# liuyuan-pal/Gen6D

Measured on AMD Instinct MI355X. Metric: query images/sec (detect+select+3x refine), 64 ref views, higher is better.
Workload: dtype f32

## Files before the change

### gen6d_amd/csrc/corr16_geom.h

```cpp
#pragma once
#include "conv16w_geom.h"

namespace corr16g {

constexpr int BM = c16g::BM;
constexpr int NW = 11;
constexpr int STAGE = 42 * 1024;
constexpr int PIECE = 1024;
constexpr int NPL = STAGE / PIECE;
constexpr int TAP_BYTES = 2048;
constexpr int RING = 3;
constexpr int RED_LD = 33;
constexpr int LDS_BYTES = 2 * STAGE;
static_assert((STAGE / 64 + 15) / 16 <= NPL, "the largest patch pick_tile admits (STAGE / 64 rows) fits NPL pieces");
static_assert(4 * BM * RED_LD * 4 <= LDS_BYTES, "the final reduction's four partial tiles fit the two stages");

struct Tile { int tw_log2, tiles_x, tpi, swa, swd; };
C16G_HD Tile pick_tile(int H, int W, int K) {
  double best = 1e30; int btw = 0;
  for (int tw = 32; tw >= 4; tw >>= 1) {
    const int th = BM / tw;
    if ((th + K - 1) * (tw + K - 1) > STAGE / 64) continue;
    const double waste = (double)((W + tw - 1) / tw * tw) * ((H + th - 1) / th * th) / ((double)W * H);
    if (waste < best - 1e-9) { best = waste; btw = tw; }
  }
  if (!btw) return {-1, 0, 0, 0, 0};
  int l2 = 0; while ((1 << l2) < btw) ++l2;
  const int th = BM / btw, tx = (W + btw - 1) / btw;
  return {l2, tx, tx * ((H + th - 1) / th), btw == 32 ? 2 : (btw == 16 ? 1 : 0), btw <= 8 ? 1 : 0};
}

struct Patch { int tw_log2, K, swa, swd, PW, P, NI; };
C16G_HD Patch patch_of(int tw_log2, int K, int swa, int swd) {
  const int PW = (1 << tw_log2) + K - 1, P = ((BM >> tw_log2) + K - 1) * PW;
  return {tw_log2, K, swa, swd, PW, P, (P + 15) >> 4};
}
struct Origin { int n, y0, x0; };
C16G_HD Origin tile_origin(const Patch& g, int tiles_x, int tpi, int t) {
  const int n = t / tpi, r = t - n * tpi, ty = r / tiles_x, tx = r - ty * tiles_x;
  return {n, ty * (BM >> g.tw_log2), tx * (1 << g.tw_log2)};
}

struct Piece { int prow, pcol, y, x, L; bool in_patch; };
C16G_HD Piece piece_of(const Patch& g, const Origin& o, int k, int lane) {
  const int q = k * 16 + (lane >> 2), R = g.K >> 1;
  const int prow = q / g.PW, pcol = q - prow * g.PW;
  return {prow, pcol, o.y0 - R + prow, o.x0 - R + pcol, (lane & 3) ^ (((pcol >> g.swa) + prow * g.swd) & 3), k < g.NI && q < g.P};
}
C16G_HD bool in_map(const Piece& pc, int H, int W) { return pc.y >= 0 && pc.y < H && pc.x >= 0 && pc.x < W; }
C16G_HD unsigned slot_bytes(int L, bool pairs, int Cin) { return pairs ? (unsigned)((L >> 1) * Cin * 2 + (L & 1) * 16) : (unsigned)(L * 16); }

C16G_HD void frag_base(const Patch& g, int r, int& qb, int& fe) {
  const int py = r >> g.tw_log2, px = r & ((1 << g.tw_log2) - 1);
  qb = (py * g.PW + px) * 64; fe = px + py * g.swd;
}
C16G_HD int tap_addr(const Patch& g, int qb, int fe, int fhalf, int ky, int kx, int stage) {
  const int so = stage * STAGE + ky * (g.PW * 64) + kx * 64, sw = ((fe + kx) >> g.swa) + ky * g.swd;
  return qb + so + (((fhalf ^ sw) & 3) << 4);
}

C16G_HD int wave_taps(int K, int wv) { return (K * K - wv + NW - 1) / NW; }
C16G_HD void first_tap(int K, int wv, int& ky, int& kx) { ky = wv / K; kx = wv - ky * K; }
C16G_HD void next_tap(int K, int& ky, int& kx) { kx += NW; while (kx >= K) { kx -= K; ++ky; } }
C16G_HD long filter_advance(int K, int wv, int& wtap) {
  wtap += NW;
  if (wtap < K * K) return NW * TAP_BYTES;
  const long d = (long)(K * K - wtap + NW + wv) * TAP_BYTES;
  wtap = wv;
  return d;
}

}
```

### gen6d_amd/csrc/detector.hip

```cpp
#include "g6d_common.h"

namespace {

struct LevelStats { float mu[3], sigma[3]; };

__global__ void assemble_kernel(const float* __restrict__ s0, const float* __restrict__ s1, const float* __restrict__ s2,
                                int hc, int wc, int rfn, LevelStats st, float clip, int hs, int ws, int scale_idx,
                                int nch, float* __restrict__ stacked) {
  const long long total = (long long)hs * ws * rfn;
  const long long i = blockIdx.x * (long long)blockDim.x + threadIdx.x;
  if (i >= total) return;
  s0 += (size_t)blockIdx.y * hc * wc * rfn; s1 += (size_t)blockIdx.y * (hc >> 1) * (wc >> 1) * rfn;
  s2 += (size_t)blockIdx.y * (hc >> 2) * (wc >> 2) * rfn; stacked += (size_t)blockIdx.y * total * nch;
  const int r = (int)(i % rfn); const int pix = (int)(i / rfn);
  const int x = pix % ws, y = pix / ws;
  const float ry = (float)hc / (float)hs, rx = (float)wc / (float)ws;
  float sy = ry * (y + 0.5f) - 0.5f; if (sy < 0.f) sy = 0.f;
  float sx = rx * (x + 0.5f) - 0.5f; if (sx < 0.f) sx = 0.f;
  const int y0 = (int)sy, x0 = (int)sx;
  const int y1 = y0 + (y0 < hc - 1), x1 = x0 + (x0 < wc - 1);
  const float ly = sy - y0, lx = sx - x0, hy = 1.f - ly, hx = 1.f - lx;
  const float* src[3] = {s0, s1, s2};
  float* dst = stacked + ((size_t)pix * rfn + r) * nch + 3 * scale_idx;
#pragma unroll
  for (int l = 0; l < 3; ++l) {
    const int wl = wc >> l;
    const float mu = st.mu[l], sg = st.sigma[l];
    auto tap = [&](int yy, int xx) {
      float v = src[l][((size_t)(yy >> l) * wl + (xx >> l)) * rfn + r];
      v = (v - mu) / sg;
      return fminf(fmaxf(v, -clip), clip);
    };
    dst[l] = hy * (hx * tap(y0, x0) + lx * tap(y0, x1)) + ly * (hx * tap(y1, x0) + lx * tap(y1, x1));
  }
}

__device__ __forceinline__ int enc_f(float f) { int b = __float_as_int(f); return b >= 0 ? b : b ^ 0x7fffffff; }
__device__ __forceinline__ float dec_f(int b) { return __int_as_float(b >= 0 ? b : b ^ 0x7fffffff); }

template <int NCH>
__global__ void __launch_bounds__(256) score_mlp_max_kernel(const float* __restrict__ stacked, int P, int rfn,
                                                            const float* __restrict__ w0, const float* __restrict__ b0,
                                                            const float* __restrict__ w1, const float* __restrict__ b1,
                                                            float* __restrict__ out, int ppb) {
  extern __shared__ int smax[];
  const int pl = threadIdx.x / rfn, r = threadIdx.x % rfn;
  const int pix = blockIdx.x * ppb + pl;
  for (int i = threadIdx.x; i < ppb * 64; i += 256) smax[i] = enc_f(-INFINITY);
  __syncthreads();
  if (pl < ppb && pix < P) {
    float in[NCH];
    const float* src = stacked + ((size_t)pix * rfn + r) * NCH;
#pragma unroll
    for (int k = 0; k < NCH; ++k) in[k] = src[k];
    typedef float f2 __attribute__((ext_vector_type(2)));
    static_assert(NCH % 2 == 0, "channel pairs");
    f2 inp[NCH / 2];
#pragma unroll
    for (int k = 0; k < NCH / 2; ++k) inp[k] = f2{in[2 * k], in[2 * k + 1]};
    f2 hp[32];
#pragma unroll
    for (int o = 0; o < 64; ++o) {
      f2 a = {b0[o], 0.f};
#pragma unroll
      for (int k = 0; k < NCH / 2; ++k) a = __builtin_elementwise_fma(inp[k], *reinterpret_cast<const f2*>(w0 + o * NCH + 2 * k), a);
      const float v = fmaxf(a.x + a.y, 0.f);
      if (o & 1) hp[o >> 1].y = v; else hp[o >> 1].x = v;
    }
    for (int o = 0; o < 64; ++o) {
      f2 a = {b1[o], 0.f};
#pragma unroll
      for (int k = 0; k < 32; ++k) a = __builtin_elementwise_fma(hp[k], *reinterpret_cast<const f2*>(w1 + o * 64 + 2 * k), a);
      atomicMax(&smax[pl * 64 + o], enc_f(a.x + a.y));
    }
  }
  __syncthreads();
  for (int i = threadIdx.x; i < ppb * 64; i += 256) {
    const int p2 = blockIdx.x * ppb + i / 64;
    if (p2 < P) out[(size_t)p2 * 64 + (i & 63)] = dec_f(smax[i]);
  }
}

__global__ void __launch_bounds__(256) decode_kernel(const float* __restrict__ scores, int ld_s,
                                                     const float* __restrict__ offset, int ld_o,
                                                     const float* __restrict__ scale, int ld_c, int hs, int ws,
                                                     float pool_ratio, float* __restrict__ result) {
  __shared__ float bv[256];
  __shared__ int bi[256];
  const int n = hs * ws;
  scores += (size_t)blockIdx.x * n * ld_s; offset += (size_t)blockIdx.x * n * ld_o; scale += (size_t)blockIdx.x * n * ld_c;
  result += blockIdx.x * 5;
  float best = -INFINITY; int idx = 0x7fffffff;
  for (int i = threadIdx.x; i < n; i += 256) {
    float v = scores[(size_t)i * ld_s];
    if (v > best || (v == best && i < idx)) { best = v; idx = i; }
  }
  bv[threadIdx.x] = best; bi[threadIdx.x] = idx;
  __syncthreads();
  for (int s = 128; s > 0; s >>= 1) {
    if (threadIdx.x < s) {
      float v = bv[threadIdx.x + s]; int j = bi[threadIdx.x + s];
      if (v > bv[threadIdx.x] || (v == bv[threadIdx.x] && j < bi[threadIdx.x])) { bv[threadIdx.x] = v; bi[threadIdx.x] = j; }
    }
    __syncthreads();
  }
  if (threadIdx.x == 0) {
    const int id = bi[0] == 0x7fffffff ? 0 : bi[0];
    const int x = id % ws, y = id / ws;
    result[0] = ((float)x + offset[(size_t)id * ld_o] + 0.5f) * pool_ratio - 0.5f;
    result[1] = ((float)y + offset[(size_t)id * ld_o + 1] + 0.5f) * pool_ratio - 0.5f;
    result[2] = exp2f(scale[(size_t)id * ld_c]);
    result[3] = (float)x; result[4] = (float)y;
  }
}


struct PyrArgs { const float* src; int planes, H, W, n; int h[4], w[4]; long long first[5]; float* dst[4]; };

#define PYR_PL 4
template <int VEC>
__global__ void resize_pyramid_kernel(const PyrArgs a) {
  const unsigned total = (unsigned)a.first[a.n];
  for (unsigned long i64 = blockIdx.x * blockDim.x + threadIdx.x; i64 < total; i64 += (unsigned long)gridDim.x * blockDim.x) {
    const unsigned i = (unsigned)i64;
    int k = 0;
#pragma unroll
    for (int j = 1; j < 4; ++j) k = (j < a.n && i >= (unsigned)a.first[j]) ? j : k;
    const unsigned l = i - (unsigned)a.first[k];
    const int h = a.h[k], w = a.w[k], wv = w / VEC;
    const int xq = (int)(l % (unsigned)wv); const unsigned t = l / (unsigned)wv;
    const int y = (int)(t % (unsigned)h), pg = (int)(t / (unsigned)h);
    const float ry = (float)a.H / (float)h, rx = (float)a.W / (float)w;
    float sy = ry * (y + 0.5f) - 0.5f; if (sy < 0.f) sy = 0.f;
    const int y0 = min((int)sy, a.H - 1);
    const int y1 = y0 + (y0 < a.H - 1);
    const float ly = sy - y0, hy = 1.f - ly;
    int x0[VEC], x1[VEC]; float lx[VEC];
#pragma unroll
    for (int e = 0; e < VEC; ++e) {
      const int x = xq * VEC + e;
      float sx = rx * (x + 0.5f) - 0.5f; if (sx < 0.f) sx = 0.f;
      x0[e] = min((int)sx, a.W - 1);
      x1[e] = x0[e] + (x0[e] < a.W - 1);
      lx[e] = sx - x0[e];
    }
    const size_t sstride = (size_t)a.H * a.W, dstride = (size_t)h * w;
    const int pl0 = pg * PYR_PL;
    const float* r0 = a.src + (size_t)pl0 * sstride + (size_t)y0 * a.W;
    const float* r1 = a.src + (size_t)pl0 * sstride + (size_t)y1 * a.W;
    float t00[PYR_PL][VEC], t01[PYR_PL][VEC], t10[PYR_PL][VEC], t11[PYR_PL][VEC];
#pragma unroll
    for (int p_ = 0; p_ < PYR_PL; ++p_) {
      const size_t o = (size_t)min(p_, a.planes - 1 - pl0) * sstride;
#pragma unroll
      for (int e = 0; e < VEC; ++e) { t00[p_][e] = r0[o + x0[e]]; t01[p_][e] = r0[o + x1[e]]; t10[p_][e] = r1[o + x0[e]]; t11[p_][e] = r1[o + x1[e]]; }
    }
    float* d = a.dst[k] + (size_t)pl0 * dstride + (size_t)y * w + xq * VEC;
#pragma unroll
    for (int p_ = 0; p_ < PYR_PL; ++p_) {
      if (pl0 + p_ >= a.planes) break;
      float v[VEC];
#pragma unroll
      for (int e = 0; e < VEC; ++e) {
        const float hx = 1.f - lx[e];
        v[e] = hy * (hx * t00[p_][e] + lx[e] * t01[p_][e]) + ly * (hx * t10[p_][e] + lx[e] * t11[p_][e]);
      }
      if constexpr (VEC == 4) *reinterpret_cast<f32x4*>(d + p_ * dstride) = f32x4{v[0], v[1], v[2], v[3]};
      else d[p_ * dstride] = v[0];
    }
  }
}
}

#define STREAM(s) reinterpret_cast<hipStream_t>(s)

extern "C" int g6d_detector_assemble(const float* s0, const float* s1, const float* s2, int hc, int wc, int rfn,
                                     const float* mu_sigma, float clip, int hs, int ws, int scale_idx, int nch,
                                     float* stacked, int batch, g6d_stream_t stream) {
  if (!s0 || !s1 || !s2 || !mu_sigma || !stacked || hc <= 0 || wc <= 0 || (hc & 3) || (wc & 3) || rfn <= 0 || hs <= 0 || ws <= 0 ||
      scale_idx < 0 || 3 * scale_idx + 3 > nch || batch < 1 || batch > 65535) {
    g6d_set_error("detector_assemble: bad args (level-0 map must be a multiple of 4, hs and ws positive)"); return G6D_EINVAL;
  }
  LevelStats st;
  for (int l = 0; l < 3; ++l) { st.mu[l] = mu_sigma[2 * l]; st.sigma[l] = mu_sigma[2 * l + 1]; }
  const long long total = (long long)hs * ws * rfn;
  hipLaunchKernelGGL(assemble_kernel, dim3((unsigned)((total + 255) / 256), batch), dim3(256), 0, STREAM(stream), s0, s1, s2, hc,
                     wc, rfn, st, clip, hs, ws, scale_idx, nch, stacked);
  return g6d_check_launch("detector_assemble");
}

extern "C" int g6d_detector_score_mlp_max(const float* stacked, int P, int rfn, int nch, const float* w0, const float* b0,
                                          const float* w1, const float* b1, float* out, g6d_stream_t stream) {
  if (!stacked || !w0 || !b0 || !w1 || !b1 || !out || P <= 0 || rfn <= 0 || rfn > 256 || nch != 12) {
    g6d_set_error("detector_score_mlp_max: bad args (rfn <= 256, nch == 12)"); return G6D_EINVAL;
  }
  const int ppb = 256 / rfn;
  hipLaunchKernelGGL(score_mlp_max_kernel<12>, dim3((P + ppb - 1) / ppb), dim3(256), (size_t)ppb * 64 * sizeof(int),
                     STREAM(stream), stacked, P, rfn, w0, b0, w1, b1, out, ppb);
  return g6d_check_launch("detector_score_mlp_max");
}

extern "C" int g6d_detector_decode(const float* scores, int ld_s, const float* offset, int ld_o, const float* scale,
                                   int ld_c, int hs, int ws, int pool_ratio, float* result, int batch, g6d_stream_t stream) {
  if (!scores || !offset || !scale || !result || hs <= 0 || ws <= 0 || batch < 1) { g6d_set_error("detector_decode: bad args"); return G6D_EINVAL; }
  hipLaunchKernelGGL(decode_kernel, dim3(batch), dim3(256), 0, STREAM(stream), scores, ld_s, offset, ld_o, scale, ld_c, hs, ws,
                     (float)pool_ratio, result);
  return g6d_check_launch("detector_decode");
}

extern "C" int g6d_resize_bilinear_pyramid(const float* src, int planes, int H, int W, int nscale, const int* hs, const int* ws,
                                           float* const* dsts, g6d_stream_t stream) {
  if (!src || !hs || !ws || !dsts || planes <= 0 || H <= 0 || W <= 0 || nscale < 1 || nscale > 4) {
    g6d_set_error("resize_bilinear_pyramid: bad args (1..4 destination sizes)"); return G6D_EINVAL;
  }
  PyrArgs a = {};
  a.src = src; a.planes = planes; a.H = H; a.W = W; a.n = nscale;
  bool vec = true;
  for (int k = 0; k < nscale; ++k)
    if (hs[k] <= 0 || ws[k] <= 0 || !dsts[k]) { g6d_set_error("resize_bilinear_pyramid: bad destination"); return G6D_EINVAL; }
    else vec = vec && (ws[k] & 3) == 0 && g6d_aligned16(dsts[k]);
  long long tot = 0;
  for (int k = 0; k < nscale; ++k) {
    a.h[k] = hs[k]; a.w[k] = ws[k]; a.dst[k] = dsts[k]; a.first[k] = tot;
    tot += (long long)((planes + PYR_PL - 1) / PYR_PL) * hs[k] * (vec ? ws[k] / 4 : ws[k]);
  }
  for (int k = nscale; k < 5; ++k) a.first[k] = tot;
  if (tot >= (1ll << 32)) { g6d_set_error("resize_bilinear_pyramid: more than 2^32 work items"); return G6D_EINVAL; }
  const long long blocks = (tot + 255) / 256;
  const dim3 grid((unsigned)(blocks < 65536 * 8 ? blocks : 65536 * 8));
  if (vec) hipLaunchKernelGGL(resize_pyramid_kernel<4>, grid, dim3(256), 0, STREAM(stream), a);
  else hipLaunchKernelGGL(resize_pyramid_kernel<1>, grid, dim3(256), 0, STREAM(stream), a);
  return g6d_check_launch("resize_bilinear_pyramid");
}
```

Measured before the change: 361.3.

## Run detector score MLP on MFMA with wave-level segmented max reduction

Rewrites the per-pixel two-layer score MLP so each wave processes 32-row tiles with 32x32x2 f32 MFMA instructions. Weights are held in registers and biases are staged in LDS. The per-pixel max over reference views is done with DPP/swizzle or shuffle-based segmented reductions before the LDS atomics, so far fewer atomics are issued. Each block now covers more pixels (up to 1024/rfn, capped at 128). The cost is heavy register use and a more complex reduction path. A live_taps helper is also added to the correlation geometry header, but nothing calls it yet.

```diff
diff --git a/gen6d_amd/csrc/corr16_geom.h b/gen6d_amd/csrc/corr16_geom.h
--- a/gen6d_amd/csrc/corr16_geom.h
+++ b/gen6d_amd/csrc/corr16_geom.h
@@ -59,6 +59,19 @@
   return qb + so + (((fhalf ^ sw) & 3) << 4);
 }
 
+struct Live { int ky0, ky1, kx0, kx1; };
+C16G_HD Live live_taps(const Patch& g, const Origin& o, int H, int W, int mt) {
+  const int R = g.K >> 1, tw = 1 << g.tw_log2;
+  const int ya = o.y0 + ((32 * mt) >> g.tw_log2), xa = o.x0 + ((32 * mt) & (tw - 1));
+  int yb = o.y0 + ((32 * mt + 31) >> g.tw_log2), xb = o.x0 + ((32 * mt + 31) & (tw - 1));
+  if (ya >= H || xa >= W) return {0, 0, 0, 0};
+  if (yb > H - 1) yb = H - 1;
+  if (xb > W - 1) xb = W - 1;
+  const int ky0 = R - yb > 0 ? R - yb : 0, ky1 = H + R - ya < g.K ? H + R - ya : g.K;
+  const int kx0 = R - xb > 0 ? R - xb : 0, kx1 = W + R - xa < g.K ? W + R - xa : g.K;
+  return {ky0, ky1, kx0, kx1};
+}
+
 C16G_HD int wave_taps(int K, int wv) { return (K * K - wv + NW - 1) / NW; }
 C16G_HD void first_tap(int K, int wv, int& ky, int& kx) { ky = wv / K; kx = wv - ky * K; }
 C16G_HD void next_tap(int K, int& ky, int& kx) { kx += NW; while (kx >= K) { kx -= K; ++ky; } }
diff --git a/gen6d_amd/csrc/detector.hip b/gen6d_amd/csrc/detector.hip
--- a/gen6d_amd/csrc/detector.hip
+++ b/gen6d_amd/csrc/detector.hip
@@ -38,47 +38,108 @@
 __device__ __forceinline__ int enc_f(float f) { int b = __float_as_int(f); return b >= 0 ? b : b ^ 0x7fffffff; }
 __device__ __forceinline__ float dec_f(int b) { return __int_as_float(b >= 0 ? b : b ^ 0x7fffffff); }
 
+template <int CTRL>
+__device__ __forceinline__ int max_dpp(int v) { return max(v, __builtin_amdgcn_update_dpp(v, v, CTRL, 0xf, 0xf, false)); }
+
 template <int NCH>
-__global__ void __launch_bounds__(256) score_mlp_max_kernel(const float* __restrict__ stacked, int P, int rfn,
+__global__ void __launch_bounds__(256, 2) score_mlp_max_kernel(const float* __restrict__ stacked, int P, int rfn,
                                                             const float* __restrict__ w0, const float* __restrict__ b0,
                                                             const float* __restrict__ w1, const float* __restrict__ b1,
                                                             float* __restrict__ out, int ppb) {
+  static_assert(NCH == 12, "layer 0 is six K pairs: channels s and 6 + s");
   extern __shared__ int smax[];
-  const int pl = threadIdx.x / rfn, r = threadIdx.x % rfn;
-  const int pix = blockIdx.x * ppb + pl;
-  for (int i = threadIdx.x; i < ppb * 64; i += 256) smax[i] = enc_f(-INFINITY);
+  float* bias = reinterpret_cast<float*>(smax + ppb * 64);
+  const int tid = threadIdx.x, lane = tid & 63, wv = __builtin_amdgcn_readfirstlane(tid >> 6), n = lane & 31, h = lane >> 5;
+  const int p0 = blockIdx.x * ppb, np = min(P - p0, ppb), nrows = np * rfn;
+  const float* rows = stacked + (size_t)p0 * rfn * NCH;
+  for (int i = tid; i < ppb * 64; i += 256) smax[i] = enc_f(-INFINITY);
+  if (tid < 128) bias[tid] = tid < 64 ? b0[tid] : b1[tid - 64];
+  auto unit = [&](int i) { return 8 * (i >> 2) + 4 * h + (i & 3); };
+  float wa[2][6], wb[2][2][16];
+#pragma unroll
+  for (int ht = 0; ht < 2; ++ht)
+#pragma unroll
+    for (int s = 0; s < 6; ++s) wa[ht][s] = w0[(32 * ht + n) * NCH + 6 * h + s];
+#pragma unroll
+  for (int ot = 0; ot < 2; ++ot)
+#pragma unroll
+    for (int ht = 0; ht < 2; ++ht)
+#pragma unroll
+      for (int i = 0; i < 16; ++i) wb[ot][ht][i] = w1[(32 * ot + n) * 64 + 32 * ht + unit(i)];
   __syncthreads();
-  if (pl < ppb && pix < P) {
-    float in[NCH];
-    const float* src = stacked + ((size_t)pix * rfn + r) * NCH;
-#pragma unroll
-    for (int k = 0; k < NCH; ++k) in[k] = src[k];
+  const int ntiles = (nrows + 31) >> 5;
+#pragma unroll 1
+  for (int t = wv; t < ntiles; t += 4) {
+    const int row = 32 * t + n;
+    const bool valid = row < nrows;
     typedef float f2 __attribute__((ext_vector_type(2)));
-    static_assert(NCH % 2 == 0, "channel pairs");
-    f2 inp[NCH / 2];
-#pragma unroll
-    for (int k = 0; k < NCH / 2; ++k) inp[k] = f2{in[2 * k], in[2 * k + 1]};
-    f2 hp[32];
-#pragma unroll
-    for (int o = 0; o < 64; ++o) {
-      f2 a = {b0[o], 0.f};
-#pragma unroll
-      for (int k = 0; k < NCH / 2; ++k) a = __builtin_elementwise_fma(inp[k], *reinterpret_cast<const f2*>(w0 + o * NCH + 2 * k), a);
-      const float v = fmaxf(a.x + a.y, 0.f);
-      if (o & 1) hp[o >> 1].y = v; else hp[o >> 1].x = v;
-    }
-    for (int o = 0; o < 64; ++o) {
-      f2 a = {b1[o], 0.f};
-#pragma unroll
-      for (int k = 0; k < 32; ++k) a = __builtin_elementwise_fma(hp[k], *reinterpret_cast<const f2*>(w1 + o * 64 + 2 * k), a);
-      atomicMax(&smax[pl * 64 + o], enc_f(a.x + a.y));
-    }
+    f2 x[3] = {{0.f, 0.f}, {0.f, 0.f}, {0.f, 0.f}};
+    if (valid) {
+      const f2* src = reinterpret_cast<const f2*>(rows + (size_t)row * NCH + 6 * h);
+#pragma unroll
+      for (int k = 0; k < 3; ++k) x[k] = src[k];
+    }
+    f32x16 hid[2], o[2];
+#pragma unroll
+    for (int ht = 0; ht < 2; ++ht)
+#pragma unroll
+      for (int i = 0; i < 16; ++i) { hid[ht][i] = bias[32 * ht + unit(i)]; o[ht][i] = bias[64 + 32 * ht + unit(i)]; }
+#pragma unroll
+    for (int s = 0; s < 6; ++s)
+#pragma unroll
+      for (int ht = 0; ht < 2; ++ht) hid[ht] = __builtin_amdgcn_mfma_f32_32x32x2f32(wa[ht][s], s & 1 ? x[s >> 1].y : x[s >> 1].x, hid[ht], 0, 0, 0);
+#pragma unroll
+    for (int ht = 0; ht < 2; ++ht)
+#pragma unroll
+      for (int i = 0; i < 16; ++i) {
+        const float hv = fmaxf(hid[ht][i], 0.f);
+#pragma unroll
+        for (int ot = 0; ot < 2; ++ot) o[ot] = __builtin_amdgcn_mfma_f32_32x32x2f32(wb[ot][ht][i], hv, o[ot], 0, 0, 0);
+      }
+    int e[2][16];
+#pragma unroll
+    for (int ot = 0; ot < 2; ++ot)
+#pragma unroll
+      for (int i = 0; i < 16; ++i) e[ot][i] = enc_f(valid ? o[ot][i] : -INFINITY);
+    const int pl = row / rfn;
+    bool head;
+    if (32 * t + 31 < nrows && (32 * t) / rfn == (32 * t + 31) / rfn) {
+#pragma unroll
+      for (int ot = 0; ot < 2; ++ot)
+#pragma unroll
+        for (int i = 0; i < 16; ++i) {
+          int v = e[ot][i];
+          v = max_dpp<0xb1>(v);
+          v = max_dpp<0x4e>(v);
+          v = max_dpp<0x141>(v);
+          v = max_dpp<0x140>(v);
+          e[ot][i] = max(v, __builtin_amdgcn_ds_swizzle(v, 0x401f));
+        }
+      head = n == 0;
+    } else {
+      for (int d = 1; d < 32; d <<= 1) {
+        if (d >= rfn) break;
+        const int pd = __shfl_down(valid ? pl : -1, d, 32);
+        const bool take = (n + d < 32) & (pd == pl);
+#pragma unroll
+        for (int ot = 0; ot < 2; ++ot)
+#pragma unroll
+          for (int i = 0; i < 16; ++i) {
+            const int other = __shfl_down(e[ot][i], d, 32);
+            if (take) e[ot][i] = max(e[ot][i], other);
+          }
+      }
+      const int before = __shfl_up(pl, 1, 32);
+      head = valid && (n == 0 || before != pl);
+    }
+    if (head)
+#pragma unroll
+      for (int ot = 0; ot < 2; ++ot)
+#pragma unroll
+        for (int i = 0; i < 16; ++i) atomicMax(&smax[pl * 64 + 32 * ot + unit(i)], e[ot][i]);
   }
   __syncthreads();
-  for (int i = threadIdx.x; i < ppb * 64; i += 256) {
-    const int p2 = blockIdx.x * ppb + i / 64;
-    if (p2 < P) out[(size_t)p2 * 64 + (i & 63)] = dec_f(smax[i]);
-  }
+  for (int i = tid; i < np * 64; i += 256) out[(size_t)p0 * 64 + i] = dec_f(smax[i]);
 }
 
 __global__ void __launch_bounds__(256) decode_kernel(const float* __restrict__ scores, int ld_s,
@@ -194,8 +255,8 @@
   if (!stacked || !w0 || !b0 || !w1 || !b1 || !out || P <= 0 || rfn <= 0 || rfn > 256 || nch != 12) {
     g6d_set_error("detector_score_mlp_max: bad args (rfn <= 256, nch == 12)"); return G6D_EINVAL;
   }
-  const int ppb = 256 / rfn;
-  hipLaunchKernelGGL(score_mlp_max_kernel<12>, dim3((P + ppb - 1) / ppb), dim3(256), (size_t)ppb * 64 * sizeof(int),
+  const int ppb = 1024 / rfn < 128 ? 1024 / rfn : 128;
+  hipLaunchKernelGGL(score_mlp_max_kernel<12>, dim3((P + ppb - 1) / ppb), dim3(256), (size_t)(ppb + 2) * 64 * sizeof(int),
                      STREAM(stream), stacked, P, rfn, w0, b0, w1, b1, out, ppb);
   return g6d_check_launch("detector_score_mlp_max");
 }
```

Result: no change. 364.1 (median of 6 runs) (+0.8%).
